# boomluo02/EEMFlow

Measured on AMD Instinct MI355X. Metric: frames/sec + EPE, EEMFlow 1280×720 dt1, 1/2/4/8 MI355X, higher is better.
Workload: dtype f32; 1 GPU; EEMFlow inference, HREM 1280x720 dt1, batch=1 per GPU (BASELINE configs[1]); synthetic 20%-dense voxel pairs resident in HBM, seeded Kaiming weights; height=720, width=1280, batch_per_gpu=1, hip_graph=True, streams_per_gpu=2, coalesced_frames=10, frames_in_flight_hint=2, preheat_steps=200, input_pairs_rotated=8, input_bytes_rotated=294912000, parallelism=replicas x1: frames sharded over ranks, no data-path collective

## Files before the change

### eemflow_amd/csrc/common.h

```cpp
#pragma once
#include <hip/hip_runtime.h>
#include <cstdio>
#include <cstdlib>
#include <stdint.h>
#include <stdio.h>

#include <type_traits>

#include "switch.h"
#include "../../include/eemflow_hip.h"

typedef float f32x2 __attribute__((ext_vector_type(2)));
typedef float f32x4 __attribute__((ext_vector_type(4)));
typedef float f32x16 __attribute__((ext_vector_type(16)));
typedef double f64x2 __attribute__((ext_vector_type(2)));
typedef unsigned u32x4 __attribute__((ext_vector_type(4)));

#define EEM_OK 0
#define EEM_ERR_ARG 1
#define EEM_ERR_HIP 2
#define EEM_ERR_STATE 3

void eem_set_error(const char* fmt, ...);

// ... 108 lines not shown
struct EncConvArgs {
    const float* in0;
    const float* in1;
    const float* wpk;
    const float* wpk2;
    const float* wwino;
    const float* zero_page;
    float* trash;
    const float* bias;
    float* out;
    int nimg;
    int nimg0;
    int hin, win;
    int hout, wout;
    int hraw, wraw;
    int pad_top, pad_left;
    int act;
    const float* gate;
    int tiles_x, tiles_y;
    float* pool_partial;
    int pool_k;
    const void* const* io;
    int io_frames = 0;
    int in_norm = 0;
    int reverse = 0;
    int nt_store = 0;
    int blocks_per_xcd = 0;
    int wino_f4 = 0;
    const float* ws2r = nullptr;
    const float* res = nullptr;
    const float* wbx3 = nullptr;
    int no_store = 0;
    int vshare = 0;
};
#define ENC_ARGS_NOW(a)                                                                                                                  \
    asm volatile("" ::"s"((a).in0), "s"((a).in1), "s"((a).wpk), "s"((a).wpk2), "s"((a).wwino), "s"((a).zero_page), "s"((a).trash),        \
                 "s"((a).bias), "s"((a).out), "s"((a).nimg), "s"((a).nimg0), "s"((a).hin), "s"((a).win), "s"((a).hout), "s"((a).wout),      \
                 "s"((a).hraw), "s"((a).wraw), "s"((a).pad_top), "s"((a).pad_left), "s"((a).act), "s"((a).gate), "s"((a).tiles_x),        \
                 "s"((a).tiles_y), "s"((a).pool_partial), "s"((a).io), "s"(gridDim.x))
int enc_conv_launch(int cin, int cout, int stride, const EncConvArgs& a, hipStream_t stream);
bool enc1_supported(const EncConvArgs& a);
int enc1_launch(const EncConvArgs& a, hipStream_t stream);
bool enc2_supported(int cin, int cout, int stride, int win);
size_t enc2_packed_floats(int cin, int cout);
void enc2_pack_weights(const float* w, int cin, int cout, float* packed);
int enc_conv2_launch(int cin, int cout, int stride, const EncConvArgs& a, hipStream_t stream);
bool s2_supported(int cin, int cout, int stride, const EncConvArgs& a);
int s2_launch(int cin, const EncConvArgs& a, hipStream_t stream);
void enc2_tile(int cin, int cout, int* th, int* tw, int* poolk);
bool s2r_shape(int cin, int cout, int stride);
size_t s2r_packed_floats(int cin, int cout);
int s2r_transform_launch(const float* w, int cin, int cout, float* packed, hipStream_t stream);
bool s2r_supported(int cin, int cout, int stride, const EncConvArgs& a);
int s2r_launch(int cin, const EncConvArgs& a, hipStream_t stream);
bool bx3_shape(int cin, int cout, int stride);
size_t bx3_packed_floats(int cin, int cout);
int bx3_transform_launch(const float* w, int cin, int cout, float* packed, hipStream_t stream);
bool bx3_supported(int cin, int cout, int stride, const EncConvArgs& a);
int bx3_launch(int cin, int stride, const EncConvArgs& a, hipStream_t stream);
bool wino_supported(int cin, int cout, int stride, int win);
size_t wino_packed_floats(int c);
int wino_transform_launch(const float* w, int c, int transpose_flip, float* packed, hipStream_t stream, int f4);
int wino_launch(int c, const EncConvArgs& a, hipStream_t stream);
void wino_tile(int c, int f4, int* th, int* tw, int* poolk);
size_t wino4_packed_floats(int c);
int wino4_transform_launch(const float* w, int c, int transpose_flip, float* packed, hipStream_t stream);
// ... 132 lines not shown
```

### eemflow_amd/csrc/conv_wino4.hip

```cpp
#include <type_traits>

#include "common.h"

namespace {

#define LDS_PTR(p) ((__attribute__((address_space(3))) void*)(p))
#define GLB_PTR(p) ((const __attribute__((address_space(1))) void*)(p))

template <int C, int NGX, int NGY>
struct W4Cfg {
    static constexpr int WAVES = 8;
    static constexpr int COG = C / 16;
    static constexpr int NG = WAVES / COG;
    static constexpr int TW = NGX * 32, TH = NGY * 8;
    static constexpr int KS = C / 4;
    static constexpr int IN_ROWS = TH + 2;
    static constexpr int ROWP = TW + 8;
    static constexpr int PPR = ROWP / 4;
    static constexpr int PC = IN_ROWS * PPR;
    static constexpr int PLANE_P = (PC + 15) / 16 * 16;
    static constexpr int PLANE = PLANE_P * 4;
    static constexpr int INP = 4 * PLANE_P;
    static constexpr int UP = COG * 9 * 64;
    static constexpr int NI = (INP + UP + 511) / 512;
    static constexpr int STAGE = NI * 2048;
    static constexpr int R = 3;
    static_assert(NG * COG == WAVES && NGX * NGY == NG, "wave roles");
    static_assert((4 * ROWP) % 64 == 32, "the two tile rows of a group must sit 128 bytes apart modulo 256 (ds_read_b128 banks)");
    static_assert((5 * ROWP + 8) * 4 < 65536, "ds_read immediate range");
};

#include "wino4_xf.h"

#ifdef EEM_STAMPS
__device__ unsigned long long g_stamps4[1024 * 8 * 128];
#define STAMP4(i) do { if (C == EEM_STAMPS && blockIdx.x < 1024 && (i) < 128) { __builtin_amdgcn_sched_barrier(0); if (lane == 0) g_stamps4[(blockIdx.x * 8 + wave) * 128 + (i)] = __builtin_amdgcn_s_memtime(); __builtin_amdgcn_sched_barrier(0); } } while (0)
#define STAMP4K(base, L) do { if ((L) < 29) STAMP4((base) + 2 * (L)); } while (0)
#else
#define STAMP4(i)
#define STAMP4K(base, L)
#endif

template <int C, int NGX, int NGY, int POOLK, int EPI, bool VS = false>
__global__ __launch_bounds__(512, 2) void wino4_kernel(EncConvArgs a) {
    ENC_ARGS_NOW(a);
    using K = W4Cfg<C, NGX, NGY>;
    constexpr int R = K::R, NI = K::NI, KS = K::KS;
    constexpr int NWX = POOLK > 0 ? K::TW / POOLK : 1;
    constexpr int RED1 = POOLK > 0 ? NGY * C * NWX : 0;
    constexpr int NSTORE = EPI == 3 ? 0 : 16;
    static_assert(EPI != 3 || POOLK > 0, "a store-free launch needs the pooling output");
    constexpr int NPOOL = POOLK > 0 ? 1 : 0;
    constexpr int RAWF = K::INP * 4, UF = K::UP * 4, VF = K::NG * 9 * 64 * 4;
    constexpr int UBASE = 3 * RAWF, VBASE = UBASE + 2 * UF;
    constexpr int RING = VS ? VBASE + 2 * VF : R * K::STAGE;
    static_assert(!VS || (K::COG == 4 && (EPI == 0 || EPI == 3) && K::INP + K::UP == NI * 512 && K::UP % 64 == 0 && KS >= 3),
                  "shared V: four waves per tile group, a piece plan without padding whose wave-instructions are all weights or all input");
    static_assert((RING + 2 * RED1) * 4 <= 160 * 1024, "LDS budget");
    static_assert(POOLK == 0 || (POOLK % 8 == 0 && K::TW % POOLK == 0 && C * NWX * NGY <= 512 && POOLK <= 32), "pool windows");
    static_assert(NI + NSTORE + NPOOL <= 63, "vmcnt immediate");
    __shared__ __attribute__((aligned(256))) float lds[RING + 2 * RED1];
    float* red0 = lds + RING;

    const int tid = threadIdx.x;
    const int lane = tid & 63;
    const int wave = __builtin_amdgcn_readfirstlane(tid >> 6);
    const int j = lane & 15, g = lane >> 4;
    const int tx = j & 7, ty = j >> 3;
    const int cog = wave % K::COG, grp = wave / K::COG;
    const int gx = grp % NGX, gy = grp / NGX;

    STAMP4(0);
#ifdef EEM_STAMPS
    const unsigned long long rt0 = __builtin_amdgcn_s_memrealtime();
#endif
    TileRange tr_ = block_tile_range(a.tiles_x * a.tiles_y * a.nimg, blockIdx.x, gridDim.x);
    int walk_stride = 1;
    if (a.reverse == 3) {
        const int T = a.tiles_x * a.tiles_y * a.nimg;
        const int cpx = (T + 7) >> 3, xcd = blockIdx.x & 7, kb = blockIdx.x >> 3, gb = gridDim.x >> 3;
        const int r0 = xcd * cpx, r1 = min(r0 + cpx, T);
        const int have = r1 - r0 - kb;
        tr_.first = r0 + kb;
        tr_.count = have > 0 ? (have + gb - 1) / gb : 0;
        walk_stride = gb;
    }
    const int ntile = tr_.count;
    if (ntile == 0) return;
    const int total = ntile * KS;
    const int T_all = a.tiles_x * a.tiles_y * a.nimg;
    auto coord_of = [&](int lt) {
        if (a.reverse == 2) return TileCoord{(lt / a.tiles_y) % a.tiles_x, lt % a.tiles_y, lt / (a.tiles_x * a.tiles_y)};
        return tile_coord(a.reverse == 1 ? T_all - 1 - lt : lt, a.tiles_x, a.tiles_y);
    };
    TileCoord cur = coord_of(tr_.first), nxt = cur, prv = cur;
    auto step_tile = [&](TileCoord& t) {
        if (a.reverse == 3) {
            t.bx += walk_stride;
            while (t.bx >= a.tiles_x) { t.bx -= a.tiles_x; if (++t.by == a.tiles_y) { t.by = 0; ++t.n; } }
        } else if (a.reverse == 2) {
            if (++t.by == a.tiles_y) { t.by = 0; if (++t.bx == a.tiles_x) { t.bx = 0; ++t.n; } }
        } else if (a.reverse == 1) tile_retreat(t, a.tiles_x, a.tiles_y);
        else tile_advance(t, a.tiles_x, a.tiles_y);
    };
    const char* zero_page = reinterpret_cast<const char*>(a.zero_page);
    const int plane_in = a.hin * a.win;

    unsigned poff[NI];
    int pryq[NI];
#pragma unroll
    for (int k = 0; k < NI; ++k) {
        const int p = VS ? (k * 8 + wave) * 64 + lane - K::UP : (k * 8 + wave) * 64 + lane;
        if (VS && p < 0) {
            poff[k] = (unsigned)(p + K::UP) * 16u;
            pryq[k] = 1 << 17;
        } else if (p < K::INP) {
            const int c = p / K::PLANE_P;
            int rem = p - c * K::PLANE_P;
            const bool pad = rem >= K::PC;
            rem = pad ? K::PC - 1 : rem;
            const int ry = rem / K::PPR, q = rem - ry * K::PPR;
            poff[k] = (unsigned)((c * a.hin + ry) * a.win + q * 4) * 4u;
            pryq[k] = ry | (q << 8) | (pad ? 1 << 16 : 0);
        } else {
            const int up = p - K::INP;
            poff[k] = (unsigned)(up < K::UP ? up : K::UP - 1) * 16u;
            pryq[k] = 1 << 17;
        }
    }
    const char* wbase = reinterpret_cast<const char*>(a.wwino);
    int dma_s = 0;
    int dma_slot = 0;
    unsigned okm = 0;
    bool dma_interior = false;
    const char* dsrc = nullptr;
    auto dma_tile = [&]() {
        const int gy0 = nxt.by * K::TH - 1, gxa = nxt.bx * K::TW - 4;
        dma_interior = gy0 >= 0 && gy0 + K::IN_ROWS <= a.hin && gxa >= 0 && gxa + K::ROWP <= a.win;
        dsrc = reinterpret_cast<const char*>(a.in0 + (size_t)nxt.n * C * plane_in) + ((long)gy0 * a.win + gxa) * 4;
        if (!dma_interior) {
            const int rymin = gy0 < 0 ? -gy0 : 0, rymax = min(K::IN_ROWS, a.hin - gy0);
            const int qmin = gxa < 0 ? (-gxa) >> 2 : 0, qmax = min(K::PPR, (a.win - gxa) >> 2);
            okm = 0;
#pragma unroll
            for (int k = 0; k < NI; ++k) {
                const int ry = pryq[k] & 0xFF, q = (pryq[k] >> 8) & 0xFF;
                const bool ok = pryq[k] >= (1 << 17) || (pryq[k] < (1 << 16) && ry >= rymin && ry < rymax && q >= qmin && q < qmax);
                okm |= ok ? 1u << k : 0u;
            }
        }
    };
    auto dma_issue = [&]() {
        float* sbase = lds + dma_slot * K::STAGE;
#ifdef EEM_DIAG
        const char* usrc = wbase + (size_t)(a.nt_store & 2 ? 0 : dma_s) * (K::UP * 16);
#else
        const char* usrc = wbase + (size_t)dma_s * (K::UP * 16);
#endif
#pragma unroll
        for (int k = 0; k < NI; ++k) {
            const bool all_in = (k + 1) * 512 <= K::INP, all_u = k * 512 >= K::INP;
            const char* gp;
            if (all_in) gp = dsrc + poff[k];
            else if (all_u) gp = usrc + poff[k];
            else gp = (pryq[k] >= (1 << 17) ? usrc : dsrc) + poff[k];
            if (!all_u && !dma_interior) gp = (okm >> k) & 1 ? gp : zero_page;
            __builtin_amdgcn_global_load_lds(GLB_PTR(gp), LDS_PTR(sbase + (k * 8 + wave) * 256), 16, 0, 0);
        }
        dsrc += (size_t)plane_in * 16;
        if (++dma_s == KS) { dma_s = 0; step_tile(nxt); dma_tile(); }
        if (++dma_slot == R) dma_slot = 0;
    };
    const bool raw_hi = (4 * 8 + wave) * 64 >= K::UP;
    auto dma_issue_vs = [&](bool do_w, bool do_raw, int ws, int uslot) {
        float* ub = lds + UBASE + uslot * UF;
        float* rb = lds + dma_slot * RAWF;
        const char* usrc = wbase + (size_t)ws * (K::UP * 16);
#pragma unroll
        for (int k = 0; k < NI; ++k) {
            const bool all_u = (k + 1) * 512 <= K::UP, all_in = k * 512 >= K::UP;
            const int pb = (k * 8 + wave) * 64;
            if (all_u || (!all_in && pb < K::UP)) {
                if (do_w) __builtin_amdgcn_global_load_lds(GLB_PTR(usrc + poff[k]), LDS_PTR(ub + pb * 4), 16, 0, 0);
            } else if (do_raw) {
                const char* gp = dsrc + poff[k];
                if (!dma_interior) gp = (okm >> k) & 1 ? gp : zero_page;
                __builtin_amdgcn_global_load_lds(GLB_PTR(gp), LDS_PTR(rb + (pb - K::UP) * 4), 16, 0, 0);
            }
        }
        if (do_raw) {
            dsrc += (size_t)plane_in * 16;
            if (++dma_s == KS) { dma_s = 0; step_tile(nxt); dma_tile(); }
            if (++dma_slot == R) dma_slot = 0;
        }
    };

    f32x4 biasq;
#pragma unroll
    for (int r = 0; r < 4; ++r) biasq[r] = a.bias[cog * 16 + g * 4 + r];

    const int lbase = g * K::PLANE + (gy * 8 + ty * 4) * K::ROWP + (gx * 8 + tx) * 4 + 2;
    const int wlbase = K::INP * 4 + (cog * 9 * 64 + lane) * 4;

    f32x4 acc[36];
    int L = 0;
    int slot = 0;

    const int prow = (a.hout + 7) >> 3;
    const bool pf_act = tid < NGY * C * NWX;
    const int pf_gy = pf_act ? tid / (C * NWX) : 0;
    const int pf_co = pf_act ? (tid - pf_gy * C * NWX) / NWX : 0, pf_wx = pf_act ? tid % NWX : 0;

    auto step = [&](auto s0_tag, auto waitn_tag) {
        constexpr bool S0 = decltype(s0_tag)::value;
        constexpr int WAITN = decltype(waitn_tag)::value;
        if (L + 1 < total) asm volatile("s_waitcnt vmcnt(%0)" ::"n"(WAITN) : "memory");
        else asm volatile("s_waitcnt vmcnt(0)" ::: "memory");
        if constexpr (S0 && POOLK > 0) asm volatile("s_waitcnt lgkmcnt(0)" ::: "memory");
        __builtin_amdgcn_s_barrier();
        STAMP4K(2, L);
        if constexpr (S0 && POOLK > 0) {
            if (L > 0) {
                const float* redp = red0 + (((L / KS) - 1) & 1) * RED1;
                const float s = redp[(pf_gy * C + pf_co) * NWX + pf_wx];
                float* pb = a.pool_partial + ((size_t)prv.n * C * prow + prv.by * NGY) * (a.tiles_x * NWX) + prv.bx * NWX;
                float* p = pf_act && prv.by * NGY + pf_gy < prow ? pb + ((size_t)pf_co * prow + pf_gy) * (a.tiles_x * NWX) + pf_wx : a.trash + lane * 4;
                *p = s;
            }
        }
        if (L + R - 1 < total) dma_issue();
        STAMP4K(64, L);

        const float* sl = lds + slot * K::STAGE;
        f32x2 t05[6], t12[6], t34[6];
        {
            const float* p = sl + lbase;
            f32x2 pout[6];
            f32x4 pmid[6];
#pragma unroll
            for (int r = 0; r < 6; ++r) {
                pout[r] = f32x2{p[r * K::ROWP + 1], p[r * K::ROWP + 6]};
                pmid[r] = *reinterpret_cast<const f32x4*>(p + r * K::ROWP + 2);
            }
            f32x2 x[6];
#pragma unroll
            for (int r = 0; r < 6; ++r) x[r] = pout[r];
            bt6(x, t05);
#pragma unroll
            for (int r = 0; r < 6; ++r) x[r] = f32x2{pmid[r][0], pmid[r][1]};
            bt6(x, t12);
#pragma unroll
            for (int r = 0; r < 6; ++r) x[r] = f32x2{pmid[r][2], pmid[r][3]};
            bt6(x, t34);
        }
        STAMP4K(65, L);
        const f32x4* wl = reinterpret_cast<const f32x4*>(sl + wlbase);
        constexpr int RB = 3;
        f32x4 wq0 = wl[0], wq1 = wl[64];
#pragma unroll
        for (int xb = 0; xb < 6; xb += RB) {
            float v[RB * 6];
#pragma unroll
            for (int xi = 0; xi < RB; ++xi) bt6_row(t05[xb + xi], t12[xb + xi], t34[xb + xi], v + xi * 6);
            __builtin_amdgcn_sched_barrier(0);
#pragma unroll
            for (int pp = 0; pp < RB * 6; ++pp) {
                const int p = xb * 6 + pp;
                if (pp > 0 && (p & 3) == 0) {
                    wq0 = wq1;
                    if ((p >> 2) + 1 < 9) wq1 = wl[((p >> 2) + 1) * 64];
                }
                if constexpr (S0) {
                    const f32x4 z = {0.f, 0.f, 0.f, 0.f};
                    acc[p] = __builtin_amdgcn_mfma_f32_16x16x4f32(wq0[p & 3], v[pp], p == 7 ? biasq : z, 0, 0, 0);
                } else {
                    acc[p] = __builtin_amdgcn_mfma_f32_16x16x4f32(wq0[p & 3], v[pp], acc[p], 0, 0, 0);
                }
            }
            __builtin_amdgcn_sched_barrier(0);
        }
        STAMP4K(3, L);
        ++L;
        slot = slot + 1 == R ? 0 : slot + 1;
    };

    auto duty_half = [&](auto h_tag, int rslot, int vslot) {
        constexpr int H = decltype(h_tag)::value;
        const float* p = lds + rslot * RAWF + lbase;
        f32x2 t05[6], t12[6], t34[6];
// ... 154 lines not shown
                        for (int x = 0; x < 4; ++x) o[yy][x] *= gt[yy][x] > 0.f ? 1.f : 0.1f;
                }
                if constexpr (EPI == 2) {
                    const char* qb = reinterpret_cast<const char*>(rsrc) + (size_t)r * hw * 4;
                    f32x4 rv[4];
#pragma unroll
                    for (int yy = 0; yy < 4; ++yy) {
                        const bool in = inx && oy + yy < a.hout;
                        rv[yy] = *reinterpret_cast<const f32x4*>(qb + (in ? lane_bo + (unsigned)yy * (unsigned)a.wout * 4u : 0u));
                    }
#pragma unroll
                    for (int yy = 0; yy < 4; ++yy)
#pragma unroll
                        for (int x = 0; x < 4; ++x) { const float t = o[yy][x] + rv[yy][x]; o[yy][x] = !(t <= 0.f) ? t : 0.f; }
                }
                float ps = 0.f;
#pragma unroll
                for (int yy = 0; yy < 4; ++yy) {
                    const bool in = inx && oy + yy < a.hout;
                    if constexpr (EPI == 3) {
                    } else if (full) {
                        if (a.nt_store) __builtin_nontemporal_store(o[yy], reinterpret_cast<f32x4*>(rb + lane_bo + (size_t)yy * a.wout * 4));
                        else *reinterpret_cast<f32x4*>(rb + lane_bo + (size_t)yy * a.wout * 4) = o[yy];
                    } else {
                        float* p = in ? reinterpret_cast<float*>(rb + lane_bo + (size_t)yy * a.wout * 4) : a.trash + lane * 4;
                        *reinterpret_cast<f32x4*>(p) = o[yy];
                    }
                    const float rs = (o[yy][0] + o[yy][1]) + (o[yy][2] + o[yy][3]);
                    ps += (full || in) ? rs : 0.f;
                }
                psum[r] = ps;
            }
        }
        if constexpr (POOLK > 0) {
            constexpr int SW = POOLK / 4;
            float* red = red0 + (it & 1) * RED1;
#pragma unroll
            for (int r = 0; r < 4; ++r) {
                const float sred = window_sum<SW>(psum[r]);
                if ((tx & (SW - 1)) == 0 && ty == 0) red[(gy * C + co0 + r) * NWX + (gx * 8 + tx) / SW] = sred;
            }
        }
    };

    using T = std::true_type;
    using F = std::false_type;
    if constexpr (VS) {
        (void)wlbase;
        dma_tile();
        dma_issue_vs(false, true, 0, 0);
        dma_issue_vs(true, false, 0, 0);
        dma_issue_vs(false, true, 0, 0);
        dma_issue_vs(false, true, 0, 0);
        if (raw_hi) asm volatile("s_waitcnt vmcnt(%0)" ::"n"(NI + 2) : "memory");
        else asm volatile("s_waitcnt vmcnt(%0)" ::"n"(NI + 1) : "memory");
        __builtin_amdgcn_s_barrier();
        make_v(0, 0);
        STAMP4(1);
        for (int it = 0; it < ntile; ++it) {
            if (it == 0) step_vs(T{}, std::integral_constant<int, 0>{});
            else step_vs(T{}, std::integral_constant<int, NSTORE>{});
#pragma unroll 1
            for (int s = 1; s < KS; ++s) step_vs(F{}, std::integral_constant<int, 0>{});
            output(it);
            if (it == 0) STAMP4(62);
            prv = cur;
            step_tile(cur);
        }
    } else {
    dma_tile();
#pragma unroll
    for (int q = 0; q < R - 1; ++q)
        if (q < total) dma_issue();
    STAMP4(1);

    for (int it = 0; it < ntile; ++it) {
        if (it == 0) {
            step(T{}, std::integral_constant<int, NI>{});
            step(F{}, std::integral_constant<int, NI>{});
        } else {
            step(T{}, std::integral_constant<int, NI + NSTORE>{});
            step(F{}, std::integral_constant<int, NI + NSTORE + NPOOL>{});
        }
#pragma unroll 1
        for (int s = 2; s < KS; ++s) step(F{}, std::integral_constant<int, NI>{});
        output(it);
        if (it == 0) STAMP4(62);
        prv = cur;
        step_tile(cur);
    }
    }
    STAMP4(60);
#ifdef EEM_STAMPS
    if (C == EEM_STAMPS && lane == 0 && blockIdx.x < 1024) g_stamps4[(blockIdx.x * 8 + wave) * 128 + 61] = __builtin_amdgcn_s_memrealtime() - rt0;
#endif
    if constexpr (POOLK > 0) {
        asm volatile("s_waitcnt lgkmcnt(0)" ::: "memory");
        __builtin_amdgcn_s_barrier();
        const float* redp = red0 + ((ntile - 1) & 1) * RED1;
        if (pf_act && prv.by * NGY + pf_gy < prow)
            a.pool_partial[(((size_t)prv.n * C + pf_co) * prow + prv.by * NGY + pf_gy) * (a.tiles_x * NWX) + prv.bx * NWX + pf_wx] =
                redp[(pf_gy * C + pf_co) * NWX + pf_wx];
    }
}

struct W4WtJobs { const float* w[W4_WT_JOBS]; float* out[W4_WT_JOBS]; int c[W4_WT_JOBS]; int flip[W4_WT_JOBS]; };
__global__ void wino4_wt_kernel(W4WtJobs jobs) {
    const float* __restrict__ w = jobs.w[blockIdx.y];
    float* __restrict__ out = jobs.out[blockIdx.y];
    const int c = jobs.c[blockIdx.y], transpose_flip = jobs.flip[blockIdx.y];
    const int t = blockIdx.x * blockDim.x + threadIdx.x;
    if (t >= c * c) return;
    const int co = t / c, ci = t - co * c;
    float gk[3][3];
    for (int ky = 0; ky < 3; ++ky)
        for (int kx = 0; kx < 3; ++kx)
            gk[ky][kx] = transpose_flip ? w[((size_t)ci * c + co) * 9 + (2 - ky) * 3 + (2 - kx)]
                                        : w[((size_t)co * c + ci) * 9 + ky * 3 + kx];
    const float G[6][3] = {{0.25f, 0.f, 0.f},
                           {-1.f / 6.f, -1.f / 6.f, -1.f / 6.f},
                           {-1.f / 6.f, 1.f / 6.f, -1.f / 6.f},
                           {1.f / 24.f, 1.f / 12.f, 1.f / 6.f},
                           {1.f / 24.f, -1.f / 12.f, 1.f / 6.f},
                           {0.f, 0.f, 1.f}};
    double m[6][3];
    for (int xi = 0; xi < 6; ++xi)
        for (int kx = 0; kx < 3; ++kx)
            m[xi][kx] = (double)G[xi][0] * gk[0][kx] + (double)G[xi][1] * gk[1][kx] + (double)G[xi][2] * gk[2][kx];
    const int ncog = c / 16;
// ... 17 lines not shown
    using K = W4Cfg<C, W::NGX, W::NGY>;
    EncConvArgs a = a0;
    a.tiles_x = ceil_div(a.wout, K::TW);
    a.tiles_y = ceil_div(a.hout, K::TH);
    const int T = a.tiles_x * a.tiles_y * a.nimg;
    int per_xcd = ceil_div(T, 8);
    static const int env_cap = enc_blocks_per_xcd(C == 16 ? "F16" : (C == 32 ? "F32" : "F64"), 0);
    int cap = env_cap > 0 ? env_cap : 32;
    if (env_cap <= 0 && a.blocks_per_xcd > 0 && C == 16 && per_xcd > 16) cap = (per_xcd + 1) / 2;
    if (per_xcd > cap) per_xcd = cap;
    if (a.pool_partial != nullptr && a.pool_k != W::POOLK) {
        eem_set_error("wino4: fused pooling with k=%d is not built for C=%d", a.pool_k, C);
        return EEM_ERR_ARG;
    }
    EEM_NOTE_GRID(per_xcd * 8, 512);
    EEM_NOTE_PIPE(2);
    if ((a.gate != nullptr || a.res != nullptr) && (a.pool_partial != nullptr || (a.gate != nullptr && a.res != nullptr))) {
        eem_set_error("wino4: gate / residual epilogues come without pooling and one at a time");
        return EEM_ERR_ARG;
    }
    if constexpr (C == 64) {
        if (a.vshare && a.gate == nullptr && a.res == nullptr) {
            if (a.pool_partial != nullptr && a.no_store)
                hipLaunchKernelGGL((wino4_kernel<C, W::NGX, W::NGY, W::POOLK, 3, true>), dim3(per_xcd * 8), dim3(512), 0, stream, a);
            else if (a.pool_partial != nullptr)
                hipLaunchKernelGGL((wino4_kernel<C, W::NGX, W::NGY, W::POOLK, 0, true>), dim3(per_xcd * 8), dim3(512), 0, stream, a);
            else
                hipLaunchKernelGGL((wino4_kernel<C, W::NGX, W::NGY, 0, 0, true>), dim3(per_xcd * 8), dim3(512), 0, stream, a);
            EEM_HIP_CHECK(hipGetLastError());
            EEM_NOTE_VARIANT(1);
            return EEM_OK;
        }
    }
    if (a.pool_partial != nullptr && a.no_store && C == 64)
        hipLaunchKernelGGL((wino4_kernel<C, W::NGX, W::NGY, W::POOLK, (C == 64 ? 3 : 0)>), dim3(per_xcd * 8), dim3(512), 0, stream, a);
    else if (a.pool_partial != nullptr)
        hipLaunchKernelGGL((wino4_kernel<C, W::NGX, W::NGY, W::POOLK, 0>), dim3(per_xcd * 8), dim3(512), 0, stream, a);
    else if (a.gate != nullptr)
        hipLaunchKernelGGL((wino4_kernel<C, W::NGX, W::NGY, 0, 1>), dim3(per_xcd * 8), dim3(512), 0, stream, a);
    else if (a.res != nullptr)
        hipLaunchKernelGGL((wino4_kernel<C, W::NGX, W::NGY, 0, 2>), dim3(per_xcd * 8), dim3(512), 0, stream, a);
    else
        hipLaunchKernelGGL((wino4_kernel<C, W::NGX, W::NGY, 0, 0>), dim3(per_xcd * 8), dim3(512), 0, stream, a);
    EEM_HIP_CHECK(hipGetLastError());
    return EEM_OK;
}

}

#ifdef EEM_STAMPS
extern "C" __attribute__((visibility("default"))) int eemflow_debug_read_stamps4(unsigned long long* dst, size_t n) {
    return hipMemcpyFromSymbol(dst, HIP_SYMBOL(g_stamps4), n * sizeof(unsigned long long)) == hipSuccess ? 0 : 2;
}
extern "C" __attribute__((visibility("default"))) int eemflow_debug_clear_stamps4() {
    static unsigned long long zero[1024 * 8 * 128];
    return hipMemcpyToSymbol(HIP_SYMBOL(g_stamps4), zero, sizeof zero) == hipSuccess ? 0 : 2;
}
#endif

size_t wino4_packed_floats(int c) { return (size_t)36 * c * c; }

int wino4_transform_multi_launch(const float* const* w, const int* c, const int* transpose_flip, float* const* packed, int njobs,
                                 hipStream_t stream) {
    EEM_REQUIRE(njobs >= 1 && njobs <= W4_WT_JOBS, "wino4_transform_multi_launch: njobs=%d", njobs);
    W4WtJobs J;
    int cmax = 0;
// ... 31 lines not shown
```

### eemflow_amd/csrc/schedule.hip

```cpp
#include "ctx.h"

bool s2r_wanted() { return sw_on<SW_EEM_S2R>(); }
bool bx3_wanted(int l) {
    const EncLayerDesc& d = kEncLayers[l];
    return d.stride == 2 || bx3_s1_wanted(d.cin);
}
bool dec_wnc_wanted(const eemflow_ctx* c, int gw, int batch) {
    const char* e = sw_raw<SW_EEM_DEC_WNC>();
    if (c->dec_wnc == nullptr || gw % 4 != 0 || (e && e[0] == '0')) return false;
    return (e && e[0] == '1') || batch >= 4;
}
static bool w4_vshare_wanted(int cin) {
    const char* e = sw_raw<SW_EEM_W4_VSHARE>();
    return cin == 64 && !(e && e[0] == '0');
}
static bool tail_head_lds_wanted(const Shape& s, const TailHeadArgs& ha) {
    const char* e = sw_raw<SW_EEM_TAIL_HEAD_LDS>();
    if (s.stream || !tail_head_lds_supported(ha) || (e && e[0] == '0')) return false;
    return (e && e[0] == '1') || s.batch >= 4;
}

static void enc_walk(const eemflow_ctx* c, const Shape& s, int layer, EncConvArgs& a) {
    a.reverse = 0;
    static_assert(kSwitches[SW_EEM_COLWALK].dflt == ((1 << ENC_3_2) | (1 << ENC_3_3)), "switches.def.h: EEM_COLWALK's default");
    const int cw = sw_int_once<SW_EEM_COLWALK>();
    if (s.enc_batch >= 2 && ((cw >> layer) & 1)) a.reverse = 2;
    static_assert(kSwitches[SW_EEM_WALK3].dflt == ((1 << ENC_1_2) | (1 << ENC_2_2) | (1 << ENC_2_3) | (1 << ENC_3_2) | (1 << ENC_3_3)), "switches.def.h: EEM_WALK3's default");
    const int w3 = sw_int_once<SW_EEM_WALK3>();
    if (s.enc_batch >= 2 && ((w3 >> layer) & 1)) a.reverse = 3;
    a.nt_store = 0;
    static const int kInFlightBlocks[ENC_NUM] = {12, 24, 0, 29, 29, 0, 0, 0};
    a.blocks_per_xcd = c->frames_in_flight >= 3 ? kInFlightBlocks[layer] : 0;
}

#ifndef EEM_DIAG
bool Hook::skipped(const char*) { return false; }
#else
bool Hook::skipped(const char* name) {
    static const std::string list = [] {
        const char* e = sw_raw_once<SW_EEM_SKIP_KERNELS>();
        if (e && e[0]) fprintf(stderr, "eemflow_hip: EEM_SKIP_KERNELS=\"%s\" is set - the launches it names are skipped and the flow is GARBAGE (diagnostic runs only)\n", e);
        return std::string(e ? e : "");
    }();
    if (list.empty()) return false;
    size_t pos = 0;
    while (pos <= list.size()) {
        size_t end = list.find(';', pos);
// ... 204 lines not shown
        a.wpk = c->arena + c->enc_w[sp.layer];
        a.wpk2 = c->enc_has2[sp.layer] ? c->arena + c->enc_w2[sp.layer] : nullptr;
        a.wwino = nullptr;
        a.wino_f4 = 0;
        if (c->use_wino && c->enc_wino[sp.layer] && (rc = ensure_wino(c, sp.layer, 0, s.enc_batch, hk.st, &a.wwino, &a.wino_f4)) != EEM_OK) return rc;
        a.ws2r = nullptr;
        if (c->enc_s2r[sp.layer] && s2r_wanted() && (rc = ensure_s2r(c, sp.layer, hk.st, &a.ws2r)) != EEM_OK) return rc;
        a.wbx3 = nullptr;
        if (c->enc_bx3[sp.layer] && bx3_wanted(sp.layer) && (rc = ensure_bx3(c, sp.layer, hk.st, &a.wbx3)) != EEM_OK) return rc;
        a.zero_page = c->zero_page;
        a.trash = c->zero_page + 256;
        a.bias = c->arena + c->enc_b[sp.layer];
        a.out = sp.out;
        a.nimg = n2; a.nimg0 = sp.layer == ENC_1_1 ? s.nimg0 : n2;
        a.hin = sp.hin; a.win = sp.win; a.hout = sp.hout; a.wout = sp.wout;
        a.hraw = sp.layer == ENC_1_1 ? s.in_h : sp.hin;
        a.wraw = sp.layer == ENC_1_1 ? s.in_w : sp.win;
        a.pad_top = sp.layer == ENC_1_1 ? c->pad[2] : 0;
        a.pad_left = sp.layer == ENC_1_1 ? c->pad[0] : 0;
        if (sp.layer == ENC_1_1 && prepadded != nullptr) {
            a.in0 = prepadded;
            a.in1 = prepadded + (size_t)s.batch * c->cin0 * s.hp * s.wp;
            a.hraw = s.hp; a.wraw = s.wp; a.pad_top = 0; a.pad_left = 0;
        }
        a.act = 1;
        a.gate = nullptr;
        a.pool_partial = nullptr;
        a.pool_k = 0;
        a.io = sp.layer == ENC_1_1 ? io : nullptr;
        a.io_frames = (sp.layer == ENC_1_1 && io != nullptr) ? c->cur_io_frames : 0;
        a.in_norm = (sp.layer == ENC_1_1 && c->deferred_norm && prepadded == nullptr) ? 1 : 0;
        a.no_store = 0;
        a.vshare = w4_vshare_wanted(d.cin) ? 1 : 0;
        enc_walk(c, s, sp.layer, a);
        for (int k = 0; k < 3; ++k)
            if (s.fuse[k] && sp.layer == (k == 0 ? ENC_1_2 : k == 1 ? ENC_2_3 : ENC_3_3)) {
                a.pool_partial = c->ppart[k].p;
                a.pool_k = k == 0 ? 32 : k == 1 ? 16 : 8;
                if (k == 2 && may_skip_store) a.no_store = 1;
            }
        const double opix = (double)n2 * sp.hout * sp.wout;
        const double flops = 2.0 * opix * d.cout * d.cin * 9;
        const double ipix = sp.layer == ENC_1_1 ? (double)n2 * s.in_h * s.in_w : (double)n2 * sp.hin * sp.win;
        const double bytes = 4.0 * (ipix * d.cin + opix * d.cout + (double)d.cout * d.cin * 9 + d.cout);
        rc = hk.run(sp.name, flops, bytes,
                    [&](hipStream_t st) { return enc_conv_launch(d.cin, d.cout, d.stride, a, st); });
        if (rc != EEM_OK) return rc;
    }
    return EEM_OK;
}

int run_enc12(eemflow_ctx* c, const Shape& s, const float* e1, const float* e2, Hook& hk, const void* const* io, const float* prepadded,
              bool* done) {
    *done = false;
    const bool off = !sw_on<SW_EEM_FUSE12>();
    if (off || s.stream || c->deferred_norm || c->keep_stage_stores || c->enc0_generic || prepadded != nullptr || !c->use_wino || !c->enc_wino[ENC_1_2] ||
        !c->layer_f4(16, s.batch) || !s.fuse[0] || c->fuse_scratch.p == nullptr)
        return EEM_OK;
    int rc;
    Enc12Args a;
    memset(&a, 0, sizeof(a));
    a.in0 = e1; a.in1 = e2; a.io = io; a.io_frames = io != nullptr ? c->cur_io_frames : 0;
    a.wpk1 = c->arena + c->enc_w[ENC_1_1]; a.bias1 = c->arena + c->enc_b[ENC_1_1];
    int f4 = 0;
    if ((rc = ensure_wino(c, ENC_1_2, 0, s.batch, hk.st, &a.u2, &f4)) != EEM_OK) return rc;
    if (!f4) return EEM_OK;
// ... 140 lines not shown
```

### eemflow_amd/csrc/switches.def.h

```cpp

SW(EEM_WINO,               INT,   1,     LOAD,  "0: direct-convolution kernels; 2: Winograd, never F(4x4)")
SW(EEM_WINO4_LAYERS,       RAW,   0,     LOAD,  "<mask>: f4_mask is always that mask (bit 0/1/2: C = 16/32/64); unset: by batch")
SW(EEM_W4_VSHARE,          RAW,   0,     CALL,  "conv_wino4.hip's shared-V form - 0: never, 1: wherever it is built (C = 64, plain / store-free epilogues of the EEMFlow forward), unset: on")
SW(EEM_S2R,                ON1,   0,     CALL,  "the stride-2 layers on conv_s2r.hip")
SW(EEM_BX3_S1,             INT,   0,     CALL,  "<mask>: stride-1 layers on conv_bx3.hip (bit 0: C = 32, 1: C = 64)")
SW(EEM_NO_BX3,             ON1,   0,     CALL,  "no layer on conv_bx3.hip")
SW(EEM_NO_S2W,             ON1,   0,     CALL,  "no layer on conv_s2.hip")
SW(EEM_S2W_64,             ON1,   0,     CALL,  "conv_s2.hip takes 32 -> 64 too")
SW(EEM_NO_ENC1,            PRESENT, 0,   CALL,  "pconv1_1 on the generic encoder kernel instead of conv_enc1.hip")
SW(EEM_V,                  FAMILY, 0,    CALL,  "EEM_V<cin>_<cout>=<index>: conv_enc2.hip's variant of that layer (100 + i: persistent variant i)")
SW(EEM_ENC_PER_XCD,        FAMILY, 0,    ONCE,  "EEM_ENC_PER_XCD[_<tag>]=<n>: blocks per XCD of the persistent encoder kernels, the tagged name first (once per launcher)")
SW(EEM_DEC_WNC,            RAW,   0,     CALL,  "decoders' conv1 / conv5 on conv_wnc.hip - 0: never, 1: at every batch, unset: from batch 4 on")
SW(EEM_TAIL_HEAD_LDS,      RAW,   0,     BUILD, "the tail head's LDS form - 0: never, 1: wherever it is supported, unset: from four frames per launch on")
SW(EEM_FUSE12,             ON1,   0,     BUILD, "pconv1_1 + pconv1_2 as one launch; also read at alloc_workspace for its block scratch")
SW(EEM_COLWALK,            INT,   192,   ONCE,  "<layer mask>: tiles in columns (default: ENC_3_2, ENC_3_3)")
SW(EEM_WALK3,              INT,   218,   ONCE,  "<layer mask>: interleaved tile walk, supersedes EEM_COLWALK (default: every stride-1 layer but pconv1_1)")
SW(EEM_NO_WNC,             ON1,   0,     CALL,  "wnc_supported is false everywhere")
SW(EEM_WNC_SMALL_MAXPX,    LONG,  30000, CALL,  "maps below it take conv_wnc.hip's 4 x 32 block tile")
SW(EEM_NO_TAIL_MULTI,      ON1,   0,     CALL,  "the small-grid conv never takes several tiles per block")
SW(EEM_SKIP_KERNELS,       RAW,   0,     ONCE,  "\"prefix;prefix\": launches skipped by name (the flow is garbage)")
SW(EEM_SKIP_SPIN_US,       FLOAT, 0,     ONCE,  "a skipped launch holds its place in the stream that long (once per launch site, Hook::run)")
SW(EEM_SKIP_SPIN_BLOCKS,   INT,   1,     ONCE,  "blocks of the place-holder launch (x 576 threads)")
SW(EEM_SKIP_SPIN_CODE,     ON1,   0,     ONCE,  "the place-holder walks code instead of sleeping")
SW(EEM_SPANS,              ON1,   0,     ONCE,  "encoder / tail chain spans to stderr every 64 frames")
SW(EEM_E12_DBG,            INT,   0,     CALL,  "enc12_kernel - 1: no phase A, 2: no phase B, 4: A's stores to the trash page, 8: A without MFMAs")
SW(EEM_WG_DBG,             INT,   0,     ONCE,  "copied to the wgrad kernels' debug word (once per launcher instantiation)")
SW(EEM_GB_DBG,             INT,   0,     ONCE,  "copied to gconvb's debug word (once per launcher instantiation)")
SW(EEM_VOX_DIRECT,         ON1,   0,     CALL,  "no banded voxelisation")
SW(EEM_VOX_BAND_FLOATS,    LONG,  0,     ONCE,  "fp64 cells per band; below 256: the site's 9216")
SW(EEM_VOX_TWOPASS,        LONG,  0,     CALL,  "<ratio>: the two-pass normalisation below that many events per voxel")
SW(EEM_IWE_EPT,            INT,   0,     CALL,  "events per binning thread, 1 / 2 / 4; else by size")
SW(EEM_IWE_DIRECT,         ON1,   0,     CALL,  "the direct (unbinned) form of the image of warped events")
SW(EEM_NO_FEWOUT,          ON1,   0,     CALL,  "no launch on the few-cout kernels")
SW(EEM_FEWOUT_SMALL_BLOCKS, LONG, 512,   ONCE,  "3 .. 8 couts: launches below that many blocks take the small form")
SW(EEM_FEWOUT_WIDE,        NOT0,  1,     CALL,  "0: the 64-pixel form for the flow head's small launches too")
SW(EEM_NO_TAPS_KERNEL,     ON1,   0,     CALL,  "no launch on the per-tap kernel")
// ... 54 lines not shown
```

### eemflow_amd/csrc/train_api.hip

```cpp
#include "ctx.h"
#include "eraft_kernels.h"
#include "train.h"

#include <vector>

namespace {

typedef eemflow_ctx::ConvRef ConvRef;

int side_stream(eemflow_ctx* c, hipStream_t st, hipStream_t* out) {
    *out = st;
    if (sw_on<SW_EEM_NO_WGRAD_STREAM>()) return EEM_OK;
    if (!c->wstream) {
        EEM_HIP_CHECK(hipStreamCreateWithFlags(&c->wstream, hipStreamNonBlocking));
        for (hipEvent_t& e : c->wev) EEM_HIP_CHECK(hipEventCreateWithFlags(&e, hipEventDisableTiming));
        EEM_HIP_CHECK(hipEventCreateWithFlags(&c->wjoin, hipEventDisableTiming));
        EEM_HIP_CHECK(hipEventCreateWithFlags(&c->prep_ev, hipEventDisableTiming));
    }
    *out = c->wstream;
    return EEM_OK;
}

const char* const kEncNames[ENC_NUM] = {"pconv1_1", "pconv1_2", "pconv2_1", "pconv2_2", "pconv2_3", "pconv3_1", "pconv3_2", "pconv3_3"};

// ... 266 lines not shown
        {ENC_1_1, c->padded.p, c->cin0, s.hp, s.wp, c->a1.p, c->g_a1.p, s.h1, s.w1, nullptr}};
    if ((rc = tr_pool_bwd_launch(c->g_pool[2].p, c->g_f13.p, (long)n2 * 64, s.h3, s.w3, 8, s.gh, s.gw, 0, c->f13.p, st)) != EEM_OK) return rc;
    bw.note("pool_3", "bwd", tr_last_form);
    for (const L& l : ls) {
        const ConvRef& r = c->t_enc[l.layer];
        if (!l.gx) {
            const bool side = sw_on_once<SW_EEM_WGRAD_LAST_SIDE>();
            hipStream_t keep = bw.wst;
            if (!side) bw.wst = st;
            rc = bw.wgrad(kEncNames[l.layer], r, l.x, l.xc, 0, l.gy, nullptr, r.cout, 0, 1, n2, l.hin, l.win, l.hout, l.wout);
            bw.wst = keep;
            if (rc != EEM_OK) return rc;
            continue;
        }
        if ((rc = bw.wgrad(kEncNames[l.layer], r, l.x, l.xc, 0, l.gy, nullptr, r.cout, 0, 1, n2, l.hin, l.win, l.hout, l.wout)) != EEM_OK) return rc;
        if (r.fast_dgrad) {
            EncConvArgs a;
            memset(&a, 0, sizeof(a));
            a.in0 = l.gy;
            a.wpk = c->arena + r.wT_enc; a.wpk2 = c->arena + r.wT_enc2; a.bias = c->arena + r.zero_bias;
            a.wwino = nullptr;
            a.wino_f4 = 0;
            if (c->use_wino && c->enc_wino[l.layer] && (rc = ensure_wino(c, l.layer, 1, s.batch, st, &a.wwino, &a.wino_f4)) != EEM_OK) return rc;
            a.zero_page = c->zero_page; a.trash = c->zero_page + 256;
            a.out = l.gx;
            a.nimg = n2; a.nimg0 = n2;
            a.hin = l.hout; a.win = l.wout; a.hout = l.hin; a.wout = l.win; a.hraw = l.hout; a.wraw = l.wout;
            a.act = 0;
            a.gate = l.x;
            {
                const bool w3 = sw_not0_once<SW_EEM_WALK3_TRAIN>();
                if (w3 && n2 >= 4) a.reverse = 3;
            }
            if ((rc = enc_conv_launch(r.cout, r.cin, 1, a, st)) != EEM_OK) return rc;
            bw.note(kEncNames[l.layer], "dgrad", a.wwino && wino_supported(r.cout, r.cin, 1, a.win) ? (a.wino_f4 ? "wino4" : "wino2") : "direct");
        } else {
            const bool first = l.layer == ENC_2_1;
            DgradS2Args d;
            d.dy = l.gy; d.w = c->flat + r.w; d.dx = l.gx; d.gate = l.x;
            d.dpool = c->g_pool[first ? 0 : 1].p; d.pool_k = first ? 32 : 16; d.gh = s.gh; d.gw = s.gw;
            d.zero_page = c->zero_page; d.trash = c->zero_page + 256;
            d.n = n2; d.cin = r.cin; d.cout = r.cout; d.hin = l.hin; d.win = l.win; d.hout = l.hout; d.wout = l.wout;
            if ((l.layer == ENC_2_1 || l.layer == ENC_3_1) && dgrad_s2_supported(d)) {
                if ((rc = dgrad_s2_launch(d, st)) != EEM_OK) return rc;
                bw.note(kEncNames[l.layer], "dgrad", "dgrad_s2");
                continue;
            }
            if ((rc = bw.dgrad(r, l.gy, nullptr, r.cout, 0, 1, n2, l.hout, l.wout, l.hin, l.win, l.gx, r.cin, 0)) != EEM_OK) return rc;
            bw.note(kEncNames[l.layer], "dgrad", "gconv");
            if (l.layer == ENC_3_1 && (rc = tr_pool_bwd_launch(c->g_pool[1].p, c->g_f12.p, (long)n2 * 32, s.h2, s.w2, 16, s.gh, s.gw, 1, c->f12.p, st)) != EEM_OK) return rc;
            if (l.layer == ENC_2_1 && (rc = tr_pool_bwd_launch(c->g_pool[0].p, c->g_f11.p, (long)n2 * 16, s.h1, s.w1, 32, s.gh, s.gw, 1, c->f11.p, st)) != EEM_OK) return rc;
            bw.note(l.layer == ENC_3_1 ? "pool_2" : "pool_1", "bwd", tr_last_form);
        }
    }
    return EEM_OK;
}

extern "C" int eemflow_backward_forms(eemflow_ctx* c, char* dst, size_t cap) {
    EEM_REQUIRE(c && dst, "eemflow_backward_forms: NULL argument");
    EEM_REQUIRE(c->bwd_forms_len > 0, "eemflow_backward_forms: no backward has run on this context");
    EEM_REQUIRE(cap > (size_t)c->bwd_forms_len, "eemflow_backward_forms: %d characters, buffer holds %zu", c->bwd_forms_len + 1, cap);
    memcpy(dst, c->bwd_forms, (size_t)c->bwd_forms_len + 1);
    return EEM_OK;
}

struct StepZero { float* grad; double* stats; bool done; };

static int forward_train_impl(eemflow_ctx* c, const float* e1, const float* e2, int batch, int in_h, int in_w, int out_h, int out_w,
// ... 212 lines not shown
```

Before: 11140 frames/s.

## Keep C=16 Winograd weights resident in LDS, with optional per-wave pipelines

For the C=16 F(4x4) Winograd encoder layers, the transformed weights U are loaded once into LDS instead of streaming through the ring with every input slice. Two forms are added. The default form (2) keeps the block-wide barrier ring carrying only input. Form 1 gives each wave its own private input ring and pooling output, which removes the block barriers and the cross-wave pooling reduction. This cuts repeated weight traffic and synchronisation, at the cost of more LDS use and extra pool stores per wave.

```diff
diff --git a/eemflow_amd/csrc/common.h b/eemflow_amd/csrc/common.h
--- a/eemflow_amd/csrc/common.h
+++ b/eemflow_amd/csrc/common.h
@@ -164,6 +164,7 @@
     const float* wbx3 = nullptr;
     int no_store = 0;
     int vshare = 0;
+    int c16_form = 0;
 };
 #define ENC_ARGS_NOW(a)                                                                                                                  \
     asm volatile("" ::"s"((a).in0), "s"((a).in1), "s"((a).wpk), "s"((a).wpk2), "s"((a).wwino), "s"((a).zero_page), "s"((a).trash),        \
diff --git a/eemflow_amd/csrc/conv_wino4.hip b/eemflow_amd/csrc/conv_wino4.hip
--- a/eemflow_amd/csrc/conv_wino4.hip
+++ b/eemflow_amd/csrc/conv_wino4.hip
@@ -41,19 +41,30 @@
 #define STAMP4K(base, L)
 #endif
 
-template <int C, int NGX, int NGY, int POOLK, int EPI, bool VS = false>
+template <int C, int NGX, int NGY, int POOLK, int EPI, bool VS = false, int US = 0>
 __global__ __launch_bounds__(512, 2) void wino4_kernel(EncConvArgs a) {
     ENC_ARGS_NOW(a);
     using K = W4Cfg<C, NGX, NGY>;
-    constexpr int R = K::R, NI = K::NI, KS = K::KS;
+    constexpr bool PW = US == 1, WS = US == 2;
+    static_assert(US == 0 || (C == 16 && NGX == 4 && NGY == 2 && EPI == 0 && !VS && (POOLK == 32 || POOLK == 0)),
+                  "stationary U: all of it fits beside the slices; one pipeline per wave: a wave's pooling window is its own group");
+    constexpr int D_ROWS = PW ? 10 : K::IN_ROWS, D_ROWP = PW ? 40 : K::ROWP, D_PPR = D_ROWP / 4, D_PC = D_ROWS * D_PPR;
+    constexpr int D_PLANE_P = (D_PC + 15) / 16 * 16, D_PLANE = D_PLANE_P * 4, D_INP = 4 * D_PLANE_P;
+    static_assert((4 * D_ROWP) % 64 == 32 && (PW || (D_PLANE_P == K::PLANE_P && D_INP == K::INP)), "slice layout");
+    constexpr int PW_UF = 36 * C * C;
+    constexpr int PW_SLOTF = D_INP * 4;
+    static_assert(!PW || D_INP % 64 == 0, "a private slot is whole wave-instructions");
+    constexpr int R = PW ? 2 : K::R, NI = PW ? D_INP / 64 : WS ? (K::INP + 511) / 512 : K::NI, KS = K::KS;
+    constexpr int STAGE_F = WS ? NI * 2048 : K::STAGE;
+    constexpr int RING_BASE = WS ? PW_UF : 0;
     constexpr int NWX = POOLK > 0 ? K::TW / POOLK : 1;
-    constexpr int RED1 = POOLK > 0 ? NGY * C * NWX : 0;
+    constexpr int RED1 = POOLK > 0 && !PW ? NGY * C * NWX : 0;
     constexpr int NSTORE = EPI == 3 ? 0 : 16;
     static_assert(EPI != 3 || POOLK > 0, "a store-free launch needs the pooling output");
-    constexpr int NPOOL = POOLK > 0 ? 1 : 0;
+    constexpr int NPOOL = POOLK > 0 ? (PW ? 4 : 1) : 0;
     constexpr int RAWF = K::INP * 4, UF = K::UP * 4, VF = K::NG * 9 * 64 * 4;
     constexpr int UBASE = 3 * RAWF, VBASE = UBASE + 2 * UF;
-    constexpr int RING = VS ? VBASE + 2 * VF : R * K::STAGE;
+    constexpr int RING = PW ? PW_UF + K::WAVES * R * PW_SLOTF : VS ? VBASE + 2 * VF : RING_BASE + R * STAGE_F;
     static_assert(!VS || (K::COG == 4 && (EPI == 0 || EPI == 3) && K::INP + K::UP == NI * 512 && K::UP % 64 == 0 && KS >= 3),
                   "shared V: four waves per tile group, a piece plan without padding whose wave-instructions are all weights or all input");
     static_assert((RING + 2 * RED1) * 4 <= 160 * 1024, "LDS budget");
@@ -110,16 +121,16 @@
     int pryq[NI];
 #pragma unroll
     for (int k = 0; k < NI; ++k) {
-        const int p = VS ? (k * 8 + wave) * 64 + lane - K::UP : (k * 8 + wave) * 64 + lane;
+        const int p = PW ? k * 64 + lane : VS ? (k * 8 + wave) * 64 + lane - K::UP : WS ? min((k * 8 + wave) * 64 + lane, D_INP - 1) : (k * 8 + wave) * 64 + lane;
         if (VS && p < 0) {
             poff[k] = (unsigned)(p + K::UP) * 16u;
             pryq[k] = 1 << 17;
-        } else if (p < K::INP) {
-            const int c = p / K::PLANE_P;
-            int rem = p - c * K::PLANE_P;
-            const bool pad = rem >= K::PC;
-            rem = pad ? K::PC - 1 : rem;
-            const int ry = rem / K::PPR, q = rem - ry * K::PPR;
+        } else if (p < D_INP) {
+            const int c = p / D_PLANE_P;
+            int rem = p - c * D_PLANE_P;
+            const bool pad = rem >= D_PC;
+            rem = pad ? D_PC - 1 : rem;
+            const int ry = rem / D_PPR, q = rem - ry * D_PPR;
             poff[k] = (unsigned)((c * a.hin + ry) * a.win + q * 4) * 4u;
             pryq[k] = ry | (q << 8) | (pad ? 1 << 16 : 0);
         } else {
@@ -135,12 +146,12 @@
     bool dma_interior = false;
     const char* dsrc = nullptr;
     auto dma_tile = [&]() {
-        const int gy0 = nxt.by * K::TH - 1, gxa = nxt.bx * K::TW - 4;
-        dma_interior = gy0 >= 0 && gy0 + K::IN_ROWS <= a.hin && gxa >= 0 && gxa + K::ROWP <= a.win;
+        const int gy0 = nxt.by * K::TH - 1 + (PW ? gy * 8 : 0), gxa = nxt.bx * K::TW - 4 + (PW ? gx * 32 : 0);
+        dma_interior = gy0 >= 0 && gy0 + D_ROWS <= a.hin && gxa >= 0 && gxa + D_ROWP <= a.win;
         dsrc = reinterpret_cast<const char*>(a.in0 + (size_t)nxt.n * C * plane_in) + ((long)gy0 * a.win + gxa) * 4;
         if (!dma_interior) {
-            const int rymin = gy0 < 0 ? -gy0 : 0, rymax = min(K::IN_ROWS, a.hin - gy0);
-            const int qmin = gxa < 0 ? (-gxa) >> 2 : 0, qmax = min(K::PPR, (a.win - gxa) >> 2);
+            const int rymin = gy0 < 0 ? -gy0 : 0, rymax = min(D_ROWS, a.hin - gy0);
+            const int qmin = gxa < 0 ? (-gxa) >> 2 : 0, qmax = min(D_PPR, (a.win - gxa) >> 2);
             okm = 0;
 #pragma unroll
             for (int k = 0; k < NI; ++k) {
@@ -151,7 +162,20 @@
         }
     };
     auto dma_issue = [&]() {
-        float* sbase = lds + dma_slot * K::STAGE;
+        if constexpr (PW) {
+            float* sbase = lds + PW_UF + (wave * R + dma_slot) * PW_SLOTF;
+#pragma unroll
+            for (int k = 0; k < NI; ++k) {
+                const char* gp = dsrc + poff[k];
+                if (!dma_interior) gp = (okm >> k) & 1 ? gp : zero_page;
+                __builtin_amdgcn_global_load_lds(GLB_PTR(gp), LDS_PTR(sbase + k * 256), 16, 0, 0);
+            }
+            dsrc += (size_t)plane_in * 16;
+            if (++dma_s == KS) { dma_s = 0; step_tile(nxt); dma_tile(); }
+            if (++dma_slot == R) dma_slot = 0;
+            return;
+        }
+        float* sbase = lds + RING_BASE + dma_slot * STAGE_F;
 #ifdef EEM_DIAG
         const char* usrc = wbase + (size_t)(a.nt_store & 2 ? 0 : dma_s) * (K::UP * 16);
 #else
@@ -170,6 +194,12 @@
         dsrc += (size_t)plane_in * 16;
         if (++dma_s == KS) { dma_s = 0; step_tile(nxt); dma_tile(); }
         if (++dma_slot == R) dma_slot = 0;
+    };
+    auto load_u = [&]() {
+#pragma unroll
+        for (int k = 0; k < (PW_UF / 256 + 7) / 8; ++k)
+            if ((k * 8 + wave) * 256 < PW_UF)
+                __builtin_amdgcn_global_load_lds(GLB_PTR(wbase + ((k * 8 + wave) * 64 + lane) * 16), LDS_PTR(lds + (k * 8 + wave) * 256), 16, 0, 0);
     };
     const bool raw_hi = (4 * 8 + wave) * 64 >= K::UP;
     auto dma_issue_vs = [&](bool do_w, bool do_raw, int ws, int uslot) {
@@ -199,7 +229,8 @@
 #pragma unroll
     for (int r = 0; r < 4; ++r) biasq[r] = a.bias[cog * 16 + g * 4 + r];
 
-    const int lbase = g * K::PLANE + (gy * 8 + ty * 4) * K::ROWP + (gx * 8 + tx) * 4 + 2;
+    const int lbase = PW ? g * D_PLANE + ty * 4 * D_ROWP + tx * 4 + 2
+                         : g * K::PLANE + (gy * 8 + ty * 4) * K::ROWP + (gx * 8 + tx) * 4 + 2;
     const int wlbase = K::INP * 4 + (cog * 9 * 64 + lane) * 4;
 
     f32x4 acc[36];
@@ -216,10 +247,10 @@
         constexpr int WAITN = decltype(waitn_tag)::value;
         if (L + 1 < total) asm volatile("s_waitcnt vmcnt(%0)" ::"n"(WAITN) : "memory");
         else asm volatile("s_waitcnt vmcnt(0)" ::: "memory");
-        if constexpr (S0 && POOLK > 0) asm volatile("s_waitcnt lgkmcnt(0)" ::: "memory");
-        __builtin_amdgcn_s_barrier();
+        if constexpr (S0 && POOLK > 0 && !PW) asm volatile("s_waitcnt lgkmcnt(0)" ::: "memory");
+        if constexpr (!PW) __builtin_amdgcn_s_barrier();
         STAMP4K(2, L);
-        if constexpr (S0 && POOLK > 0) {
+        if constexpr (S0 && POOLK > 0 && !PW) {
             if (L > 0) {
                 const float* redp = red0 + (((L / KS) - 1) & 1) * RED1;
                 const float s = redp[(pf_gy * C + pf_co) * NWX + pf_wx];
@@ -228,10 +259,11 @@
                 *p = s;
             }
         }
-        if (L + R - 1 < total) dma_issue();
+        if constexpr (!PW)
+            if (L + R - 1 < total) dma_issue();
         STAMP4K(64, L);
 
-        const float* sl = lds + slot * K::STAGE;
+        const float* sl = PW ? lds + PW_UF + (wave * R + slot) * PW_SLOTF : lds + RING_BASE + slot * STAGE_F;
         f32x2 t05[6], t12[6], t34[6];
         {
             const float* p = sl + lbase;
@@ -239,8 +271,8 @@
             f32x4 pmid[6];
 #pragma unroll
             for (int r = 0; r < 6; ++r) {
-                pout[r] = f32x2{p[r * K::ROWP + 1], p[r * K::ROWP + 6]};
-                pmid[r] = *reinterpret_cast<const f32x4*>(p + r * K::ROWP + 2);
+                pout[r] = f32x2{p[r * D_ROWP + 1], p[r * D_ROWP + 6]};
+                pmid[r] = *reinterpret_cast<const f32x4*>(p + r * D_ROWP + 2);
             }
             f32x2 x[6];
 #pragma unroll
@@ -253,8 +285,12 @@
             for (int r = 0; r < 6; ++r) x[r] = f32x2{pmid[r][2], pmid[r][3]};
             bt6(x, t34);
         }
+        if constexpr (PW) {
+            asm volatile("s_waitcnt lgkmcnt(0)" ::: "memory");
+            if (L + R < total) dma_issue();
+        }
         STAMP4K(65, L);
-        const f32x4* wl = reinterpret_cast<const f32x4*>(sl + wlbase);
+        const f32x4* wl = reinterpret_cast<const f32x4*>(US != 0 ? lds + (L & (KS - 1)) * (PW_UF / KS) + lane * 4 : sl + wlbase);
         constexpr int RB = 3;
         f32x4 wq0 = wl[0], wq1 = wl[64];
 #pragma unroll
@@ -475,7 +511,16 @@
                 psum[r] = ps;
             }
         }
-        if constexpr (POOLK > 0) {
+        if constexpr (POOLK > 0 && PW) {
+            const bool act = j == 0 && cur.by * NGY + gy < prow;
+            float* pb = a.pool_partial + (((size_t)cur.n * C + co0) * prow + cur.by * NGY + gy) * (a.tiles_x * NWX) + cur.bx * NWX + gx;
+#pragma unroll
+            for (int r = 0; r < 4; ++r) {
+                const float sred = window_sum<POOLK / 4>(psum[r]);
+                float* p = act ? pb + (size_t)r * prow * (a.tiles_x * NWX) : a.trash + lane * 4;
+                *p = sred;
+            }
+        } else if constexpr (POOLK > 0) {
             constexpr int SW = POOLK / 4;
             float* red = red0 + (it & 1) * RED1;
 #pragma unroll
@@ -512,15 +557,27 @@
         }
     } else {
     dma_tile();
+    if constexpr (PW) {
+        dma_issue();
+        load_u();
+        dma_issue();
+        asm volatile("s_waitcnt vmcnt(%0)" ::"n"(NI) : "memory");
+        __builtin_amdgcn_s_barrier();
+    } else {
+    if constexpr (WS) load_u();
 #pragma unroll
     for (int q = 0; q < R - 1; ++q)
         if (q < total) dma_issue();
+    }
     STAMP4(1);
 
     for (int it = 0; it < ntile; ++it) {
         if (it == 0) {
             step(T{}, std::integral_constant<int, NI>{});
             step(F{}, std::integral_constant<int, NI>{});
+        } else if constexpr (PW) {
+            step(T{}, std::integral_constant<int, NI + NSTORE + NPOOL>{});
+            step(F{}, std::integral_constant<int, NI + NSTORE + NPOOL>{});
         } else {
             step(T{}, std::integral_constant<int, NI + NSTORE>{});
             step(F{}, std::integral_constant<int, NI + NSTORE + NPOOL>{});
@@ -537,7 +594,7 @@
 #ifdef EEM_STAMPS
     if (C == EEM_STAMPS && lane == 0 && blockIdx.x < 1024) g_stamps4[(blockIdx.x * 8 + wave) * 128 + 61] = __builtin_amdgcn_s_memrealtime() - rt0;
 #endif
-    if constexpr (POOLK > 0) {
+    if constexpr (POOLK > 0 && !PW) {
         asm volatile("s_waitcnt lgkmcnt(0)" ::: "memory");
         __builtin_amdgcn_s_barrier();
         const float* redp = red0 + ((ntile - 1) & 1) * RED1;
@@ -621,6 +678,26 @@
             return EEM_OK;
         }
     }
+    if constexpr (C == 16) {
+        if (a.c16_form == 1 && a.gate == nullptr && a.res == nullptr) {
+            if (a.pool_partial != nullptr)
+                hipLaunchKernelGGL((wino4_kernel<C, W::NGX, W::NGY, W::POOLK, 0, false, 1>), dim3(per_xcd * 8), dim3(512), 0, stream, a);
+            else
+                hipLaunchKernelGGL((wino4_kernel<C, W::NGX, W::NGY, 0, 0, false, 1>), dim3(per_xcd * 8), dim3(512), 0, stream, a);
+            EEM_HIP_CHECK(hipGetLastError());
+            EEM_NOTE_VARIANT(2);
+            return EEM_OK;
+        }
+        if (a.c16_form == 2 && a.gate == nullptr && a.res == nullptr) {
+            if (a.pool_partial != nullptr)
+                hipLaunchKernelGGL((wino4_kernel<C, W::NGX, W::NGY, W::POOLK, 0, false, 2>), dim3(per_xcd * 8), dim3(512), 0, stream, a);
+            else
+                hipLaunchKernelGGL((wino4_kernel<C, W::NGX, W::NGY, 0, 0, false, 2>), dim3(per_xcd * 8), dim3(512), 0, stream, a);
+            EEM_HIP_CHECK(hipGetLastError());
+            EEM_NOTE_VARIANT(3);
+            return EEM_OK;
+        }
+    }
     if (a.pool_partial != nullptr && a.no_store && C == 64)
         hipLaunchKernelGGL((wino4_kernel<C, W::NGX, W::NGY, W::POOLK, (C == 64 ? 3 : 0)>), dim3(per_xcd * 8), dim3(512), 0, stream, a);
     else if (a.pool_partial != nullptr)
diff --git a/eemflow_amd/csrc/schedule.hip b/eemflow_amd/csrc/schedule.hip
--- a/eemflow_amd/csrc/schedule.hip
+++ b/eemflow_amd/csrc/schedule.hip
@@ -13,6 +13,11 @@
 static bool w4_vshare_wanted(int cin) {
     const char* e = sw_raw<SW_EEM_W4_VSHARE>();
     return cin == 64 && !(e && e[0] == '0');
+}
+static int w4_c16_form(int cin) {
+    const char* e = sw_raw<SW_EEM_W4_C16_WAVES>();
+    if (cin != 16 || (e && e[0] == '0')) return 0;
+    return e && e[0] == '1' ? 1 : 2;
 }
 static bool tail_head_lds_wanted(const Shape& s, const TailHeadArgs& ha) {
     const char* e = sw_raw<SW_EEM_TAIL_HEAD_LDS>();
@@ -283,6 +288,7 @@
         a.in_norm = (sp.layer == ENC_1_1 && c->deferred_norm && prepadded == nullptr) ? 1 : 0;
         a.no_store = 0;
         a.vshare = w4_vshare_wanted(d.cin) ? 1 : 0;
+        a.c16_form = w4_c16_form(d.cin);
         enc_walk(c, s, sp.layer, a);
         for (int k = 0; k < 3; ++k)
             if (s.fuse[k] && sp.layer == (k == 0 ? ENC_1_2 : k == 1 ? ENC_2_3 : ENC_3_3)) {
diff --git a/eemflow_amd/csrc/switches.def.h b/eemflow_amd/csrc/switches.def.h
--- a/eemflow_amd/csrc/switches.def.h
+++ b/eemflow_amd/csrc/switches.def.h
@@ -2,6 +2,7 @@
 SW(EEM_WINO,               INT,   1,     LOAD,  "0: direct-convolution kernels; 2: Winograd, never F(4x4)")
 SW(EEM_WINO4_LAYERS,       RAW,   0,     LOAD,  "<mask>: f4_mask is always that mask (bit 0/1/2: C = 16/32/64); unset: by batch")
 SW(EEM_W4_VSHARE,          RAW,   0,     CALL,  "conv_wino4.hip's shared-V form - 0: never, 1: wherever it is built (C = 64, plain / store-free epilogues of the EEMFlow forward), unset: on")
+SW(EEM_W4_C16_WAVES,       RAW,   0,     CALL,  "conv_wino4.hip at C = 16 (plain epilogue of the EEMFlow forward) - 0: the weights ride the ring, 1: U resident in LDS and one pipeline per wave, 2 / unset: U resident in LDS, barrier form")
 SW(EEM_S2R,                ON1,   0,     CALL,  "the stride-2 layers on conv_s2r.hip")
 SW(EEM_BX3_S1,             INT,   0,     CALL,  "<mask>: stride-1 layers on conv_bx3.hip (bit 0: C = 32, 1: C = 64)")
 SW(EEM_NO_BX3,             ON1,   0,     CALL,  "no layer on conv_bx3.hip")
diff --git a/eemflow_amd/csrc/train_api.hip b/eemflow_amd/csrc/train_api.hip
--- a/eemflow_amd/csrc/train_api.hip
+++ b/eemflow_amd/csrc/train_api.hip
@@ -322,8 +322,12 @@
                 const bool w3 = sw_not0_once<SW_EEM_WALK3_TRAIN>();
                 if (w3 && n2 >= 4) a.reverse = 3;
             }
+            eem_last_variant = 0;
             if ((rc = enc_conv_launch(r.cout, r.cin, 1, a, st)) != EEM_OK) return rc;
-            bw.note(kEncNames[l.layer], "dgrad", a.wwino && wino_supported(r.cout, r.cin, 1, a.win) ? (a.wino_f4 ? "wino4" : "wino2") : "direct");
+            const char* form = a.wwino && wino_supported(r.cout, r.cin, 1, a.win) ? (a.wino_f4 ? "wino4" : "wino2") : "direct";
+            char tagged[24];
+            if (eem_last_variant != 0) { snprintf(tagged, sizeof tagged, "%s_v%d", form, eem_last_variant); form = tagged; }
+            bw.note(kEncNames[l.layer], "dgrad", form);
         } else {
             const bool first = l.layer == ENC_2_1;
             DgradS2Args d;
```

After: 11220 frames/s (median of 5 runs). No clear change (+0.6%).
